# ArthurBrussee/brush

Measured on NVIDIA H100. Metric: fwd+bwd Mpix/s @1M Gaussians 1080p, higher is better.
Workload: dtype f32

## Files before the change

### brush_b200/csrc/api.cu

```cuda
#include <cuda_runtime.h>

#include <algorithm>
#include <cmath>
#include <cstdio>
#include <cstdint>
#include <cstring>
#include <new>

#include "bg_common.cuh"
#include "bg_project.cuh"
#include "bg_dp.cuh"
#include "bg_update.cuh"
#include "bg_refine.cuh"

namespace bg {
cudaError_t launch_project_cull(cudaStream_t, int, bool, const float *, const float *, uint32_t, const BgCamera &,
                                uint32_t, uint32_t, uint32_t, uint32_t, uint32_t *, uint32_t *, uint32_t *, float *,
                                uint32_t *, unsigned long long *, uint32_t *, unsigned long long *, const uint32_t *,
                                uint32_t);
cudaError_t launch_gather_scan(cudaStream_t, int, const uint32_t *, const uint32_t *, uint32_t, const uint32_t *,
                               uint32_t *, uint32_t *, uint32_t, uint32_t *, uint32_t *, unsigned long long *,
                               const uint32_t *, uint32_t);
cudaError_t launch_project_visible_emit(cudaStream_t, int, bool, int, const float *, const float *, const float *,
                                        const uint32_t *, const uint32_t *, const BgCamera &, uint32_t, uint32_t,
                                        float *, uint32_t *, uint32_t *, uint32_t, uint32_t *, const unsigned long long *,
                                        uint32_t *, uint32_t);
cudaError_t launch_tile_offsets(cudaStream_t, int, const uint32_t *, const uint32_t *, uint32_t, uint32_t *);
cudaError_t launch_radix_hist(cudaStream_t, int, const uint32_t *, uint32_t, const uint32_t *, uint32_t, uint32_t,
                              uint32_t *);
cudaError_t launch_onesweep_pass(cudaStream_t, int, const uint32_t *, const uint32_t *, uint32_t *, uint32_t *,
                                 uint32_t, const uint32_t *, uint32_t, uint32_t, const uint32_t *, uint32_t *,
                                 unsigned long long *, unsigned long long *, const uint32_t *, uint32_t);
cudaError_t launch_bump_epoch(cudaStream_t, uint32_t *);
uint64_t sort_max_tiles(uint64_t n);
cudaError_t launch_blend_fwd(cudaStream_t, bool, bool, uint32_t, const float *, const uint32_t *, uint32_t *, const uint32_t *,
                             void *, float *, uint32_t *, uint32_t *, uint32_t, uint32_t, uint32_t, const float *, const float *,
                             float *);
cudaError_t launch_blend_bwd(cudaStream_t, bool, uint32_t, const float *, const uint32_t *, const uint32_t *, const float *,
                             const float *, const uint32_t *, const uint32_t *, float *, unsigned long long *, uint32_t,
                             uint32_t, uint32_t, const float *, const float *, const float *, const float *, float *);
cudaError_t launch_project_bwd(cudaStream_t, bool, int, const float *, const float *, const float *,
                               const uint32_t *, const float *, uint32_t, const BgCamera &, float *, float *, float *,
                               float *, float *);
cudaError_t launch_depth_to_means(cudaStream_t, const uint32_t *, const float *, uint32_t, const BgCamera &, float *);
cudaError_t launch_normal_noise(cudaStream_t, uint64_t, uint64_t, uint64_t, float *);
cudaError_t launch_train_fill_lr(cudaStream_t, float *, float *, uint32_t, float, float, float, float);
cudaError_t launch_loss_reduce(cudaStream_t, const float *, uint32_t, uint32_t, const float *, float *);
cudaError_t launch_min_scale(cudaStream_t, uint32_t, const float *, const float *, uint32_t, float, float *);
cudaError_t launch_fold_min_scale_fwd(cudaStream_t, uint32_t, const float *, const float *, const float *, float *, float *);
// ... 31 lines not shown
    snprintf(g_err, sizeof(g_err), "%s: %s", what, e == cudaSuccess ? "invalid argument" : cudaGetErrorString(e));
}

#define BG_CUDA(call)                          \
    do {                                       \
        cudaError_t e__ = (call);              \
        if (e__ != cudaSuccess) {              \
            set_err(#call, e__);               \
            return BG_ERR_CUDA;                \
        }                                      \
    } while (0)

struct BgContext {
    int device = 0;
    int sm_count = 0;
    uint32_t max_n = 0, max_w = 0, max_h = 0, max_tiles = 0;
    uint32_t max_isect = 0;
    uint32_t *epoch_dev = nullptr;
    uint64_t arena_bytes = 0;
    uint32_t *ctl = nullptr;
    uint32_t *depth_key[2] = {nullptr, nullptr};
    uint32_t *depth_val[2] = {nullptr, nullptr};
    uint32_t *counts = nullptr, *cum = nullptr, *cgid_from_gid = nullptr;
    unsigned long long *hit_masks = nullptr;
    float *projected = nullptr;
    uint32_t *isect_key[2] = {nullptr, nullptr};
    uint32_t *isect_val[2] = {nullptr, nullptr};
    uint32_t *tile_offsets = nullptr;
    uint32_t *live_masks = nullptr, *warp_batches = nullptr;
    unsigned long long *blend_stats = nullptr;
    unsigned long long *lb_scan = nullptr;
    unsigned long long *lb_sort = nullptr;
    uint64_t lb_scan_words = 0, lb_sort_words = 0, lb_sort_tile_words = 0;
    uint32_t *counters_host = nullptr;
    int depth_out = 0, isect_out = 0;
    bool depth_forward = false;
};

enum EpochSlots : uint32_t { EP_PROJECT = 0, EP_DEPTH_SORT = 1 , EP_SCAN = 5, EP_TILE_SORT = 6  };

extern "C" uint32_t bg_abi_version(void) { return BG_ABI_VERSION; }
extern "C" const char *bg_last_error_string(void) { return g_err; }

template <typename T>
static cudaError_t arena_alloc(BgContext *c, T **p, uint64_t count) {
    uint64_t bytes = std::max<uint64_t>(count, 1) * sizeof(T);
    bytes = (bytes + 255) & ~uint64_t(255);
    cudaError_t e = cudaMalloc((void **)p, bytes);
    if (e == cudaSuccess) c->arena_bytes += bytes;
    return e;
}

extern "C" int32_t bg_ctx_destroy(BgContext *c) {
    if (!c) return BG_ERR_NULL;
    cudaSetDevice(c->device);
    void *ptrs[] = {c->ctl, c->depth_key[0], c->depth_key[1], c->depth_val[0], c->depth_val[1], c->counts, c->cum,
                    c->cgid_from_gid, c->hit_masks, c->projected, c->isect_key[0], c->isect_key[1], c->isect_val[0], c->isect_val[1],
                    c->tile_offsets, c->lb_scan, c->lb_sort, c->epoch_dev, c->live_masks, c->warp_batches, c->blend_stats};
    for (void *p : ptrs)
        if (p) cudaFree(p);
    if (c->counters_host) cudaFreeHost(c->counters_host);
    delete c;
    return BG_OK;
}

extern "C" int32_t bg_ctx_create(int32_t device, uint32_t max_splats, uint32_t max_w, uint32_t max_h,
                                 uint64_t max_intersections, BgContext **out_ctx) {
    if (!out_ctx) return BG_ERR_NULL;
    *out_ctx = nullptr;
    if (max_splats == 0 || max_w == 0 || max_h == 0) { set_err("bg_ctx_create: zero capacity", cudaSuccess); return BG_ERR_INVALID; }
    if (max_intersections == 0) max_intersections = std::max<uint64_t>(16ull * max_splats, 1ull << 22);
    if (max_intersections >= (1ull << 31)) { set_err("bg_ctx_create: max_intersections must be < 2^31", cudaSuccess); return BG_ERR_INVALID; }
    BG_CUDA(cudaSetDevice(device));
    BgContext *c = new (std::nothrow) BgContext();
    if (!c) return BG_ERR_CUDA;
    c->device = device;
    c->max_n = max_splats; c->max_w = max_w; c->max_h = max_h;
    c->max_isect = (uint32_t)max_intersections;
    c->max_tiles = ((max_w + TILE_W - 1) / TILE_W) * ((max_h + TILE_W - 1) / TILE_W);
    cudaDeviceProp prop;
    cudaError_t e = cudaGetDeviceProperties(&prop, device);
    if (e != cudaSuccess) { set_err("cudaGetDeviceProperties", e); delete c; return BG_ERR_CUDA; }
    c->sm_count = prop.multiProcessorCount;
    const uint64_t n = max_splats, I = c->max_isect;
    const uint64_t sort_tiles = sort_max_tiles(std::max<uint64_t>(n, I));
    c->lb_sort_tile_words = sort_tiles * 256;
    c->lb_sort_words = c->lb_sort_tile_words + (sort_tiles / 16 + 2) * 256;
    c->lb_scan_words = (n + 255) / 256 + 64;
    bool ok = true;
    ok = ok && arena_alloc(c, &c->ctl, 2 * CTL_WORDS) == cudaSuccess;
    for (int i = 0; i < 2; i++) {
        ok = ok && arena_alloc(c, &c->depth_key[i], n) == cudaSuccess;
        ok = ok && arena_alloc(c, &c->depth_val[i], n) == cudaSuccess;
        ok = ok && arena_alloc(c, &c->isect_key[i], I) == cudaSuccess;
        ok = ok && arena_alloc(c, &c->isect_val[i], I) == cudaSuccess;
    }
    ok = ok && arena_alloc(c, &c->counts, n) == cudaSuccess;
    ok = ok && arena_alloc(c, &c->cum, n) == cudaSuccess;
    ok = ok && arena_alloc(c, &c->cgid_from_gid, n) == cudaSuccess;
    ok = ok && arena_alloc(c, &c->hit_masks, n) == cudaSuccess;
    ok = ok && arena_alloc(c, &c->projected, n * BG_PROJECTED_STRIDE) == cudaSuccess;
    ok = ok && arena_alloc(c, &c->tile_offsets, (uint64_t)c->max_tiles * 2) == cudaSuccess;
    ok = ok && arena_alloc(c, &c->live_masks, (I / 32 + c->max_tiles + 2) * 4) == cudaSuccess;
    ok = ok && arena_alloc(c, &c->warp_batches, (uint64_t)c->max_tiles * 4) == cudaSuccess;
    ok = ok && arena_alloc(c, &c->blend_stats, 4) == cudaSuccess;
    ok = ok && arena_alloc(c, &c->lb_scan, c->lb_scan_words) == cudaSuccess;
    ok = ok && arena_alloc(c, &c->lb_sort, c->lb_sort_words) == cudaSuccess;
    ok = ok && arena_alloc(c, &c->epoch_dev, 1) == cudaSuccess;
    ok = ok && cudaHostAlloc((void **)&c->counters_host, 16 * sizeof(uint32_t), cudaHostAllocDefault) == cudaSuccess;
    if (ok) {
        ok = cudaMemset(c->lb_scan, 0, c->lb_scan_words * 8) == cudaSuccess &&
             cudaMemset(c->lb_sort, 0, c->lb_sort_words * 8) == cudaSuccess &&
             cudaMemset(c->ctl, 0, 2 * CTL_WORDS * 4) == cudaSuccess &&
             cudaMemset(c->epoch_dev, 0, 4) == cudaSuccess;
    }
    if (!ok) {
        set_err("bg_ctx_create: arena allocation", cudaGetLastError());
        bg_ctx_destroy(c);
        return BG_ERR_CUDA;
    }
    memset(c->counters_host, 0, 16 * sizeof(uint32_t));
    *out_ctx = c;
    return BG_OK;
// ... 35 lines not shown
    const int deg = sh_degree_from_k(k);
    if (deg < 0) { set_err("Invalid nr. of sh bases", cudaSuccess); return BG_ERR_INVALID; }
    if (pass < 0 || pass > 2) { set_err("invalid pass", cudaSuccess); return BG_ERR_INVALID; }
    if (cam->camera_model > BG_CAMERA_THIN_PRISM_FISHEYE) return BG_ERR_UNSUPPORTED;
    const bool bwd_info = pass != BG_PASS_FORWARD;
    if (bwd_info && n > 0 && !visible) return BG_ERR_NULL;
    if ((((uintptr_t)transforms) | ((uintptr_t)sh) | ((uintptr_t)raw_opac) | ((uintptr_t)out_img)) & 15u) {
        set_err("bg_render_forward: arrays must be 16-byte aligned (bulk / 128-bit access)", cudaSuccess);
        return BG_ERR_INVALID;
    }
    const uint32_t tiles_x = (w + TILE_W - 1) / TILE_W, tiles_y = (h + TILE_W - 1) / TILE_W;
    const uint32_t num_tiles = tiles_x * tiles_y;
    if (n > c->max_n || num_tiles > c->max_tiles) { set_err("bg_render_forward: exceeds context capacity", cudaSuccess); return BG_ERR_CAPACITY; }
    cudaStream_t s = (cudaStream_t)stream;
    BG_CUDA(cudaSetDevice(c->device));
    c->depth_forward = out_depth != nullptr;

    BG_CUDA(launch_bump_epoch(s, c->epoch_dev));
    BG_CUDA(cudaMemsetAsync(c->ctl, 0, CTL_WORDS * sizeof(uint32_t), s));
    BG_CUDA(cudaMemsetAsync(c->tile_offsets, 0, (size_t)num_tiles * 2 * sizeof(uint32_t), s));
    if (bwd_info && n > 0) BG_CUDA(cudaMemsetAsync(visible, 0, (size_t)n * sizeof(float), s));

    const int pgrid = c->sm_count * 5;
    const int vgrid = c->sm_count * 6;
    uint32_t *counters = c->ctl + CTL_COUNTERS;
    BG_CUDA(launch_project_cull(s, pgrid, mip != 0, transforms, raw_opac, n, *cam, w, h, tiles_x, tiles_y,
                                c->depth_key[0], c->depth_val[0], c->counts, max_radius, c->cgid_from_gid, c->hit_masks, c->ctl,
                                c->lb_scan, c->epoch_dev, EP_PROJECT));
    int dout = 0;
    {
        int32_t r = run_sort(c, s, c->depth_key[0], c->depth_val[0], c->depth_key, c->depth_val, n, counters + 0, 32,
                             c->ctl + CTL_HIST_DEPTH, c->ctl + CTL_TICKETS + TK_DEPTH_HIST, 1, EP_DEPTH_SORT, &dout,
                             true);
        if (r != BG_OK) return r;
    }
    c->depth_out = dout;
    const uint32_t *gid_sorted = c->depth_val[dout];
    BG_CUDA(launch_gather_scan(s, c->sm_count * 2, c->counts, gid_sorted, n, counters + 0, c->cum, counters + 1,
                               c->max_isect, counters + 2, c->ctl + CTL_TICKETS + TK_SCAN, c->lb_scan, c->epoch_dev, EP_SCAN));
    uint32_t bits = 0;
    while (bits < 32 && (num_tiles >> bits) != 0) bits++;
    if (n > 0)
        BG_CUDA(launch_project_visible_emit(s, vgrid, mip != 0, deg, transforms, sh, raw_opac, gid_sorted, c->cum, *cam,
                                            tiles_x, tiles_y, c->projected, c->isect_key[0], c->isect_val[0],
                                            c->max_isect, c->cgid_from_gid, c->hit_masks, c->ctl, bits));
    int iout = 0;
    {
        const uint32_t passes = (bits + 7) / 8;
        const int first_dst = 1;
        int32_t r = run_sort(c, s, c->isect_key[0], c->isect_val[0], c->isect_key, c->isect_val, c->max_isect,
                             counters + 1, bits, c->ctl + CTL_HIST_TILE, c->ctl + CTL_TICKETS + TK_TILE_HIST, first_dst,
                             EP_TILE_SORT, &iout, n > 0 && bits <= 16);
        if (r != BG_OK) return r;
        (void)passes;
    }
    c->isect_out = iout;
    BG_CUDA(launch_tile_offsets(s, c->sm_count * 16, c->isect_key[iout], c->ctl, num_tiles, c->tile_offsets));
    BG_CUDA(launch_blend_fwd(s, bwd_info, pass == BG_PASS_BACKWARD_SMOOTH, num_tiles, c->projected, c->isect_val[iout],
                             c->tile_offsets, gid_sorted, out_img, visible, c->live_masks, c->warp_batches, tiles_x, w, h, bg,
                             reinterpret_cast<const float *>(c->depth_key[dout]), out_depth));
    BG_CUDA(cudaMemcpyAsync(c->counters_host, counters, 4 * sizeof(uint32_t), cudaMemcpyDeviceToHost, s));

    st->projected = c->projected;
    st->compact_gid_from_isect = c->isect_val[iout];
    st->global_from_compact_gid = gid_sorted;
    st->compact_from_global_gid = c->cgid_from_gid;
    st->tile_offsets = c->tile_offsets;
    st->depths = reinterpret_cast<const float *>(c->depth_key[dout]);
// ... 1009 lines not shown
```

### brush_b200/csrc/project.cu

```cuda
#include "bg_project.cuh"

namespace bg {

constexpr int PROJ_THREADS = 256;

struct CullResult {
    bool visible;
    float depth;
    uint32_t tiles;
    float radius;
    unsigned long long mask;
    float mx, my, c00, c01, c11, pt;
    uint32_t min_x, min_y, bbw, ntiles;
};

template <bool MIP, bool DIST>
__device__ __forceinline__ CullResult cull_one(const float *t, float raw_opac, const BgCamera &u, uint32_t img_w,
                                               uint32_t img_h, uint32_t tiles_x, uint32_t tiles_y) {
    CullResult r;
    r.visible = false; r.depth = 0.0f; r.tiles = 0; r.radius = 0.0f; r.mask = 0ull;
    r.mx = r.my = r.c00 = r.c01 = r.c11 = r.pt = 0.0f;
    r.min_x = r.min_y = r.bbw = r.ntiles = 0;
    V3 mean_c = world_to_cam(mk3(t[0], t[1], t[2]), u);
    if (!(is_finite(mean_c) && mean_c.z <= 1.0e10f)) return r;
    if (!in_front<DIST>(mean_c, u)) return r;
    V3 scl = mk3(det_expf(t[7]), det_expf(t[8]), det_expf(t[9]));
    if (!is_finite(scl)) return r;
    Q4 qu; qu.w = t[3]; qu.x = t[4]; qu.y = t[5]; qu.z = t[6];
    float qn = dot(qu, qu);
    if (!(qn >= 1.0e-6f && is_finite(qn))) return r;
    if (!is_finite(raw_opac)) return r;
    Q4 quat = normalize(qu);
    S2 raw_cov = calc_cov2d<DIST>(scl, quat, mean_c, u);
    float comp;
    S2 cov = compensate_cov2d<MIP>(raw_cov, comp);
    float opac = det_sigmoid(raw_opac) * comp;
    if (!is_finite(cov)) return r;
    float mx, my;
    project_mean<DIST>(mean_c, u, mx, my);
    if (!(opac >= 1.0f / 255.0f)) return r;
    float pt = det_logf(opac * 255.0f);
    S2 conic = inverse(cov);
    float ex, ey;
    bbox_extent(conic, pt, ex, ey);
    if (!(ex >= 0.0f && ey >= 0.0f)) return r;
    float wf = (float)img_w, hf = (float)img_h;
    bool on_screen = mx + ex > 0.0f && mx - ex < wf && my + ey > 0.0f && my - ey < hf;
    if (!on_screen) return r;
    TileBox bb = tile_bbox(mx, my, ex, ey, tiles_x, tiles_y);
    r.visible = true;
    r.depth = mean_c.z;
    r.radius = fmaxf(ex / wf, ey / hf);
    r.mx = mx; r.my = my; r.c00 = conic.c00; r.c01 = conic.c01; r.c11 = conic.c11; r.pt = pt;
    r.min_x = bb.min_x; r.min_y = bb.min_y; r.bbw = bb.max_x - bb.min_x;
    r.ntiles = (bb.max_y - bb.min_y) * r.bbw;
    return r;
}

__device__ __forceinline__ void warp_count_tiles(CullResult &r) {
    const uint32_t lane = threadIdx.x & 31u;
    uint32_t incl = r.ntiles;
    for (int o = 1; o < 32; o <<= 1) {
        uint32_t t = __shfl_up_sync(0xffffffffu, incl, o);
        if (lane >= (uint32_t)o) incl += t;
    }
    const uint32_t pre = incl - r.ntiles;
    const uint32_t total = __shfl_sync(0xffffffffu, incl, 31);
    uint32_t hits_count = 0;
    unsigned long long mask = 0ull;
    for (uint32_t base = 0; base < total; base += 32) {
        const uint32_t j = base + lane;
        uint32_t own = 0;
#pragma unroll
        for (int step = 16; step > 0; step >>= 1) {
            uint32_t cand = own + step;
            uint32_t pc = __shfl_sync(0xffffffffu, pre, cand & 31u);
// ... 7 lines not shown
        conic.c11 = __shfl_sync(0xffffffffu, r.c11, own);
        const float pt = __shfl_sync(0xffffffffu, r.pt, own);
        const uint32_t min_x = __shfl_sync(0xffffffffu, r.min_x, own), min_y = __shfl_sync(0xffffffffu, r.min_y, own);
        const uint32_t bbw = __shfl_sync(0xffffffffu, r.bbw, own);
        bool hit = false;
        if (j < total) {
            const uint32_t ry = local / bbw, rx = local - ry * bbw;
            hit = tile_hit(min_x + rx, min_y + ry, mx, my, conic, pt);
        }
        const uint32_t hits = __ballot_sync(0xffffffffu, hit);
        const uint32_t lo = max(pre, base), hi = min(pre + r.ntiles, base + 32u);
        if (hi > lo) {
            const uint32_t sft = lo - base, len = hi - lo;
            const uint32_t seg = (hits >> sft) & (len >= 32u ? 0xffffffffu : ((1u << len) - 1u));
            hits_count += __popc(seg);
            const uint32_t local0 = lo - pre;
            if (local0 < 64u) mask |= (unsigned long long)seg << local0;
        }
    }
    r.tiles = hits_count;
    r.mask = mask;
}

template <bool MIP, bool DIST>
__global__ void __launch_bounds__(PROJ_THREADS)
project_cull_kernel(const float *__restrict__ transforms, const float *__restrict__ raw_opac, uint32_t n,
                    BgCamera u, uint32_t img_w, uint32_t img_h, uint32_t tiles_x, uint32_t tiles_y,
                    uint32_t *__restrict__ depth_keys, uint32_t *__restrict__ gids,
                    uint32_t *__restrict__ counts_by_gid, float *__restrict__ max_radius,
                    uint32_t *__restrict__ cgid_from_gid, unsigned long long *__restrict__ hit_masks,
                    uint32_t *__restrict__ ctl,
                    unsigned long long *__restrict__ lb_state, const uint32_t *__restrict__ epoch_base, uint32_t epoch_off) {
    const uint32_t epoch = ((*epoch_base) * 32u + epoch_off) & 0x3FFFFFFFu;
    __shared__ __align__(128) float s_rows_buf[2][PROJ_THREADS * 10];
    __shared__ __align__(8) unsigned long long s_bar[2];
    __shared__ uint32_t s_scan[33];
    __shared__ uint32_t s_tile, s_tile_next, s_prefix;
    __shared__ uint32_t s_dhist[4 * 256];
    const uint32_t num_tiles = (n + PROJ_THREADS - 1) / PROJ_THREADS;
    if (threadIdx.x == 0) { mbar_init(&s_bar[0], 1); mbar_init(&s_bar[1], 1); }
    for (uint32_t i = threadIdx.x; i < 4 * 256; i += PROJ_THREADS) s_dhist[i] = 0;
    __syncthreads();
    auto issue = [&](uint32_t t, uint32_t b) {
        const uint32_t tb = t * PROJ_THREADS;
        const uint32_t bytes = (min((uint32_t)PROJ_THREADS, n - tb) * 40u) & ~15u;
        mbar_expect_tx(&s_bar[b], bytes);
        tma_bulk_g2s(s_rows_buf[b], transforms + (size_t)tb * 10, bytes, &s_bar[b]);
    };
    if (threadIdx.x == 0) {
        uint32_t t = atomicAdd(&ctl[CTL_TICKETS + TK_PROJECT], 1u);
        s_tile = t;
        if (t < num_tiles) issue(t, 0);
    }
    __syncthreads();
    uint32_t tile = s_tile, buf = 0, phase0 = 0, phase1 = 0;
    while (tile < num_tiles) {
        if (threadIdx.x == 0) {
            uint32_t t = atomicAdd(&ctl[CTL_TICKETS + TK_PROJECT], 1u);
            s_tile_next = t;
            if (t < num_tiles) issue(t, buf ^ 1u);
        }
        const uint32_t base = tile * PROJ_THREADS;
        const uint32_t rows = min((uint32_t)PROJ_THREADS, n - base);
        float *s_rows = s_rows_buf[buf];
        if (buf == 0) { mbar_wait(&s_bar[0], phase0); phase0 ^= 1u; } else { mbar_wait(&s_bar[1], phase1); phase1 ^= 1u; }
        if (threadIdx.x == rows - 1) {
            const uint32_t nf = rows * 10, covered = ((rows * 40u) & ~15u) >> 2;
            for (uint32_t i = covered; i < nf; i++) s_rows[i] = __ldg(transforms + (size_t)base * 10 + i);
        }
        const uint32_t gid = base + threadIdx.x;
        CullResult r;
        r.visible = false; r.depth = 0.0f; r.tiles = 0; r.radius = 0.0f; r.mask = 0ull;
        r.mx = r.my = r.c00 = r.c01 = r.c11 = r.pt = 0.0f;
        r.min_x = r.min_y = r.bbw = r.ntiles = 0;
        if (threadIdx.x < rows) {
            float t[10];
#pragma unroll
            for (int j = 0; j < 10; j++) t[j] = s_rows[threadIdx.x * 10 + j];
            r = cull_one<MIP, DIST>(t, __ldg(raw_opac + gid), u, img_w, img_h, tiles_x, tiles_y);
            max_radius[gid] = r.radius;
            cgid_from_gid[gid] = 0xFFFFFFFFu;
        }
        uint32_t total;
        uint32_t local = block_exclusive_scan(r.visible ? 1u : 0u, s_scan, &total);
        unsigned long long *st = lb_state + tile;
        if (threadIdx.x == 0) lb_store(st, epoch, tile == 0 ? LB_INCLUSIVE : LB_AGGREGATE, total);
        warp_count_tiles(r);
        if (threadIdx.x < 32) {
            uint32_t prefix = (tile == 0) ? 0u : lb_lookback_warp(lb_state, tile, epoch);
            if (threadIdx.x == 0) {
                if (tile != 0) lb_store(st, epoch, LB_INCLUSIVE, prefix + total);
                s_prefix = prefix;
                if (tile == num_tiles - 1) ctl[CTL_COUNTERS + 0] = prefix + total;
            }
        }
        __syncthreads();
        if (r.visible) {
            uint32_t slot = s_prefix + local;
            const uint32_t dk = __float_as_uint(r.depth);
            depth_keys[slot] = dk;
#pragma unroll
            for (int p = 0; p < 4; p++) atomicAdd(&s_dhist[p * 256 + ((dk >> (8 * p)) & 255u)], 1u);
            gids[slot] = gid;
            counts_by_gid[gid] = r.tiles;
            hit_masks[gid] = r.mask;
        }
        tile = s_tile_next;
        buf ^= 1u;
        __syncthreads();
    }
    uint32_t *hist = ctl + CTL_HIST_DEPTH;
    for (uint32_t i = threadIdx.x; i < 4 * 256; i += PROJ_THREADS) {
        const uint32_t c = s_dhist[i];
        if (c) atomicAdd(&hist[i], c);
    }
}

constexpr int SCAN_THREADS = 256, SCAN_ITEMS = 8, SCAN_TILE = SCAN_THREADS * SCAN_ITEMS;

__global__ void __launch_bounds__(SCAN_THREADS)
gather_scan_kernel(const uint32_t *__restrict__ in, const uint32_t *__restrict__ gather_idx ,
                   uint32_t n_host, const uint32_t *__restrict__ n_dev, uint32_t *__restrict__ out,
                   uint32_t *__restrict__ total_out , uint32_t capacity,
                   uint32_t *__restrict__ overflow_flag , uint32_t *__restrict__ ticket,
                   unsigned long long *__restrict__ lb_state, const uint32_t *__restrict__ epoch_base, uint32_t epoch_off) {
    const uint32_t epoch = ((*epoch_base) * 32u + epoch_off) & 0x3FFFFFFFu;
    __shared__ uint32_t s_scan[33];
    __shared__ uint32_t s_tile, s_prefix;
// ... 35 lines not shown
                        tot = capacity;
                    }
                    *total_out = tot;
                }
            }
        }
        __syncthreads();
        const uint32_t off = s_prefix + excl;
#pragma unroll
        for (int i = 0; i < SCAN_ITEMS; i++) {
            uint32_t idx = base + i;
            if (idx < n) out[idx] = off + v[i];
        }
        __syncthreads();
    }
}

constexpr int VIS_THREADS = 128;

__device__ __forceinline__ void prefetch_l2_bulk(const void *p, uint32_t bytes) {
    asm volatile("cp.async.bulk.prefetch.L2.global [%0], %1;" ::"l"(p), "r"(bytes) : "memory");
}

template <bool MIP, int DEG, bool DIST>
__global__ void __launch_bounds__(VIS_THREADS, 6)
project_visible_emit_kernel(const float *__restrict__ transforms, const float *__restrict__ sh,
                            const float *__restrict__ raw_opac, const uint32_t *__restrict__ gid_sorted,
                            const uint32_t *__restrict__ cum, BgCamera u, uint32_t tiles_x, uint32_t tiles_y,
                            float *__restrict__ projected, uint32_t *__restrict__ tile_keys,
                            uint32_t *__restrict__ isect_vals, uint32_t isect_capacity,
                            uint32_t *__restrict__ cgid_from_gid, const unsigned long long *__restrict__ hit_masks,
                            uint32_t *__restrict__ ctl, uint32_t tile_bits) {
    constexpr int KF = (DEG + 1) * (DEG + 1) * 3;
    constexpr bool VEC4 = (KF % 4) == 0;
    constexpr uint32_t EMIT_BUF = 1024;
    __shared__ uint32_t s_emit_keys[(VIS_THREADS / 32) * EMIT_BUF];
    __shared__ uint8_t s_emit_own[(VIS_THREADS / 32) * EMIT_BUF];
    __shared__ uint32_t s_thist[2 * 256];
    const uint32_t hist_passes = (tile_bits <= 16u) ? (tile_bits + 7u) / 8u : 0u;
    const uint32_t hi_mask = (tile_bits > 8u) ? ((1u << min(8u, tile_bits - 8u)) - 1u) : 0u;
    const uint32_t lo_mask = (1u << min(8u, tile_bits)) - 1u;
    for (uint32_t i = threadIdx.x; i < 2 * 256; i += VIS_THREADS) s_thist[i] = 0;
    __syncthreads();
    auto count_key = [&](uint32_t key) {
        if (hist_passes > 0) atomicAdd(&s_thist[key & lo_mask], 1u);
        if (hist_passes > 1) atomicAdd(&s_thist[256 + ((key >> 8) & hi_mask)], 1u);
    };
    const uint32_t nvis = ctl[CTL_COUNTERS + 0];
    const uint32_t num_tickets = (nvis + 31u) / 32u;
    const uint32_t lane = threadIdx.x & 31u, wid = threadIdx.x >> 5;
    const uint32_t lt_mask = (1u << lane) - 1u;
    uint32_t *wkeys = s_emit_keys + wid * EMIT_BUF;
    uint8_t *wown = s_emit_own + wid * EMIT_BUF;
    auto take_ticket = [&]() {
        uint32_t t = 0;
        if (lane == 0) t = atomicAdd(&ctl[CTL_TICKETS + TK_VISIBLE], 1u);
        return __shfl_sync(0xffffffffu, t, 0);
    };
    uint32_t ticket = take_ticket();
    uint32_t gid = 0;
    if (ticket < num_tickets && ticket * 32u + lane < nvis) gid = __ldg(gid_sorted + ticket * 32u + lane);
    while (ticket < num_tickets) {
        const uint32_t cgid = ticket * 32u + lane;
        const bool active = cgid < nvis;
        const uint32_t ticket_next = take_ticket();
        const bool next_active = ticket_next < num_tickets && ticket_next * 32u + lane < nvis;
        uint32_t gid_next = 0;
        if (next_active) gid_next = __ldg(gid_sorted + ticket_next * 32u + lane);

        TileBox bb;
        bb.min_x = bb.min_y = bb.max_x = bb.max_y = 0;
        uint32_t base = 0, budget = 0;
        unsigned long long hitm = 0ull;
        float e_mx = 0.f, e_my = 0.f, e_pt = 0.f;
        S2 e_conic; e_conic.c00 = e_conic.c01 = e_conic.c11 = 0.f;
        if (active) {
            float coef[KF];
            if (VEC4) {
                const float4 *row4 = reinterpret_cast<const float4 *>(sh + (size_t)gid * KF);
#pragma unroll
                for (int i = 0; i < KF / 4; i++) {
                    float4 q = __ldg(row4 + i);
                    coef[4 * i] = q.x; coef[4 * i + 1] = q.y; coef[4 * i + 2] = q.z; coef[4 * i + 3] = q.w;
                }
            } else {
                const float *row = sh + (size_t)gid * KF;
#pragma unroll
                for (int i = 0; i < KF; i++) coef[i] = __ldg(row + i);
            }
            const float2 *t2 = reinterpret_cast<const float2 *>(transforms + (size_t)gid * 10);
            float2 a0 = __ldg(t2), a1 = __ldg(t2 + 1), a2 = __ldg(t2 + 2), a3 = __ldg(t2 + 3), a4 = __ldg(t2 + 4);
            const float ro = __ldg(raw_opac + gid);
            hitm = __ldg(hit_masks + gid);
            base = (cgid == 0) ? 0u : __ldg(cum + cgid - 1);
            budget = __ldg(cum + cgid) - base;
            V3 mean = mk3(a0.x, a0.y, a1.x);
            Q4 qu; qu.w = a1.y; qu.x = a2.x; qu.y = a2.y; qu.z = a3.x;
            V3 scl = mk3(det_expf(a3.y), det_expf(a4.x), det_expf(a4.y));
            Q4 quat = normalize(qu);
            V3 mean_c = world_to_cam(mean, u);
            S2 raw_cov = calc_cov2d<DIST>(scl, quat, mean_c, u);
            float comp;
            S2 cov = compensate_cov2d<MIP>(raw_cov, comp);
            float opac = det_sigmoid(ro) * comp;
            S2 conic = inverse(cov);
            float mx, my;
            project_mean<DIST>(mean_c, u, mx, my);
            V3 vdir = normalize(sub(mean, mk3(u.cam_pos[0], u.cam_pos[1], u.cam_pos[2])));
            V3 raw = sh_to_color<DEG>([&](int i) { return coef[i]; }, vdir);
            float cr = raw.x + 0.5f, cg = raw.y + 0.5f, cb = raw.z + 0.5f;
            cr = clampf(is_finite(cr) ? cr : 0.0f, -100.0f, 100.0f);
            cg = clampf(is_finite(cg) ? cg : 0.0f, -100.0f, 100.0f);
            cb = clampf(is_finite(cb) ? cb : 0.0f, -100.0f, 100.0f);
            float pt = det_logf(opac * 255.0f);
            float4 *dst = reinterpret_cast<float4 *>(projected + (size_t)cgid * BG_PROJECTED_STRIDE);
            const float L2E = 1.4426950408889634f;
            dst[0] = make_float4(mx, my, conic.c00, conic.c01);
            dst[1] = make_float4(conic.c11, opac, cr, cg);
            dst[2] = make_float4(cb, (0.5f * L2E) * conic.c11, (0.5f * L2E) * conic.c00, L2E * conic.c01);
            dst[3] = make_float4(pt, 0.0f, 0.0f, 0.0f);
            cgid_from_gid[gid] = cgid;
            float ex, ey;
            bbox_extent(conic, pt, ex, ey);
            bb = tile_bbox(mx, my, ex, ey, tiles_x, tiles_y);
            e_mx = mx; e_my = my; e_conic = conic; e_pt = pt;
        }
        if (next_active) {
            const char *srow = reinterpret_cast<const char *>(sh + (size_t)gid_next * KF);
            const char *trow = reinterpret_cast<const char *>(transforms + (size_t)gid_next * 10);
            if (VEC4) prefetch_l2_bulk(srow, KF * 4);
            prefetch_l2_bulk(reinterpret_cast<const char *>(reinterpret_cast<uintptr_t>(trow) & ~(uintptr_t)15), 48);
        }
        const uint32_t warp_base = __shfl_sync(0xffffffffu, base, 0);
        uint32_t end_here = active ? base + budget : 0u;
        for (int o = 16; o > 0; o >>= 1) end_here = max(end_here, __shfl_xor_sync(0xffffffffu, end_here, o));
        const uint32_t warp_total = end_here - warp_base;
        const bool staged = warp_total <= EMIT_BUF;
        const uint32_t off = base - warp_base;
        const uint32_t bbw = bb.max_x - bb.min_x, bbh = bb.max_y - bb.min_y;
        const bool big = active && bbw * bbh > 64u;
        auto put = [&](uint32_t slot_off, uint32_t slot_base, uint32_t owner_lane, uint32_t h, uint32_t key) {
            if (staged) { wkeys[slot_off + h] = key; wown[slot_off + h] = (uint8_t)owner_lane; }
            else {
                uint32_t o = slot_base + h;
                if (o < isect_capacity) { tile_keys[o] = key; isect_vals[o] = ticket * 32u + owner_lane; count_key(key); }
            }
        };
        if (active && !big) {
            uint32_t hits = 0;
            unsigned long long m = hitm;
            const unsigned long long row_mask = (bbw >= 64u) ? ~0ull : ((1ull << bbw) - 1ull);
            uint32_t row_key = bb.min_x + bb.min_y * tiles_x;
            for (uint32_t ry = 0; ry < bbh && hits < budget; ry++, m = (bbw >= 64u) ? 0ull : (m >> bbw), row_key += tiles_x) {
                unsigned long long rb = m & row_mask;
                while (rb && hits < budget) {
// ... 77 lines not shown
tile_offsets_kernel(const uint32_t *__restrict__ tile_ids, const uint32_t *__restrict__ ctl, uint32_t num_tiles,
                    uint32_t *__restrict__ tile_offsets) {
    const uint32_t n = ctl[CTL_COUNTERS + 1];
    const uint32_t groups = (n + 3u) / 4u;
    for (uint32_t g = blockIdx.x * blockDim.x + threadIdx.x; g < groups; g += gridDim.x * blockDim.x) {
        const uint32_t i0 = g * 4u;
        uint32_t v[4];
        if (i0 + 4u <= n) {
            const uint4 q = __ldg(reinterpret_cast<const uint4 *>(tile_ids) + g);
            v[0] = q.x; v[1] = q.y; v[2] = q.z; v[3] = q.w;
        } else {
#pragma unroll
            for (int e = 0; e < 4; e++) v[e] = (i0 + e < n) ? __ldg(tile_ids + i0 + e) : 0xFFFFFFFFu;
        }
        uint32_t prev = (i0 == 0) ? 0xFFFFFFFFu : __ldg(tile_ids + i0 - 1);
#pragma unroll
        for (int e = 0; e < 4; e++) {
            if (i0 + e < n) tile_boundary(i0 + e, v[e], prev, n, num_tiles, tile_offsets);
            prev = v[e];
        }
    }
}

cudaError_t launch_project_cull(cudaStream_t s, int grid, bool mip, const float *transforms, const float *raw_opac,
                                uint32_t n, const BgCamera &u, uint32_t w, uint32_t h, uint32_t tx, uint32_t ty,
                                uint32_t *depth_keys, uint32_t *gids, uint32_t *counts, float *max_radius,
                                uint32_t *cgid_from_gid, unsigned long long *hit_masks, uint32_t *ctl,
                                unsigned long long *lb, const uint32_t *epoch_base, uint32_t epoch_off) {
    if (n == 0) return cudaSuccess;
    const bool dist = u.camera_model != BG_CAMERA_PINHOLE;
#define BG_LAUNCH_CULL(M, D)                                                                                       \
    project_cull_kernel<M, D><<<grid, PROJ_THREADS, 0, s>>>(transforms, raw_opac, n, u, w, h, tx, ty, depth_keys, \
                                                            gids, counts, max_radius, cgid_from_gid, hit_masks, ctl, lb, epoch_base, epoch_off)
    if (mip) { if (dist) BG_LAUNCH_CULL(true, true); else BG_LAUNCH_CULL(true, false); }
    else     { if (dist) BG_LAUNCH_CULL(false, true); else BG_LAUNCH_CULL(false, false); }
#undef BG_LAUNCH_CULL
    return cudaGetLastError();
}

cudaError_t launch_gather_scan(cudaStream_t s, int grid, const uint32_t *in, const uint32_t *gather_idx,
                               uint32_t n_host, const uint32_t *n_dev, uint32_t *out, uint32_t *total_out,
                               uint32_t capacity, uint32_t *overflow_flag, uint32_t *ticket,
                               unsigned long long *lb, const uint32_t *epoch_base, uint32_t epoch_off) {
    if (n_host == 0) return cudaSuccess;
    gather_scan_kernel<<<grid, SCAN_THREADS, 0, s>>>(in, gather_idx, n_host, n_dev, out, total_out, capacity,
                                                     overflow_flag, ticket, lb, epoch_base, epoch_off);
    return cudaGetLastError();
}

template <bool MIP>
static cudaError_t launch_visible_deg(cudaStream_t s, int grid, int deg, const float *transforms, const float *sh,
                                      const float *raw_opac, const uint32_t *gid_sorted, const uint32_t *cum,
                                      const BgCamera &u, uint32_t tx, uint32_t ty, float *projected,
                                      uint32_t *tile_keys, uint32_t *isect_vals, uint32_t cap,
                                      uint32_t *cgid_from_gid, const unsigned long long *hit_masks, uint32_t *ctl,
                                      uint32_t tile_bits) {
    const bool dist = u.camera_model != BG_CAMERA_PINHOLE;
#define BG_LAUNCH_VIS(D)                                                                                                   \
    if (dist) project_visible_emit_kernel<MIP, D, true><<<grid, VIS_THREADS, 0, s>>>(transforms, sh, raw_opac, gid_sorted, cum, u, \
                                                                     tx, ty, projected, tile_keys, isect_vals, cap, cgid_from_gid, hit_masks, ctl, tile_bits); \
    else project_visible_emit_kernel<MIP, D, false><<<grid, VIS_THREADS, 0, s>>>(transforms, sh, raw_opac, gid_sorted, cum, u, \
                                                                     tx, ty, projected, tile_keys, isect_vals, cap, cgid_from_gid, hit_masks, ctl, tile_bits)
    switch (deg) {
        case 0: BG_LAUNCH_VIS(0); break;
        case 1: BG_LAUNCH_VIS(1); break;
        case 2: BG_LAUNCH_VIS(2); break;
        case 3: BG_LAUNCH_VIS(3); break;
        case 4: BG_LAUNCH_VIS(4); break;
        default: return cudaErrorInvalidValue;
    }
#undef BG_LAUNCH_VIS
    return cudaGetLastError();
}

cudaError_t launch_project_visible_emit(cudaStream_t s, int grid, bool mip, int deg, const float *transforms,
                                        const float *sh, const float *raw_opac, const uint32_t *gid_sorted,
                                        const uint32_t *cum, const BgCamera &u, uint32_t tx, uint32_t ty,
                                        float *projected, uint32_t *tile_keys, uint32_t *isect_vals, uint32_t cap,
                                        uint32_t *cgid_from_gid, const unsigned long long *hit_masks, uint32_t *ctl,
                                        uint32_t tile_bits) {
    return mip ? launch_visible_deg<true>(s, grid, deg, transforms, sh, raw_opac, gid_sorted, cum, u, tx, ty, projected,
                                          tile_keys, isect_vals, cap, cgid_from_gid, hit_masks, ctl, tile_bits)
               : launch_visible_deg<false>(s, grid, deg, transforms, sh, raw_opac, gid_sorted, cum, u, tx, ty,
                                           projected, tile_keys, isect_vals, cap, cgid_from_gid, hit_masks, ctl, tile_bits);
}

cudaError_t launch_tile_offsets(cudaStream_t s, int grid, const uint32_t *tile_ids, const uint32_t *ctl,
                                uint32_t num_tiles, uint32_t *tile_offsets) {
    tile_offsets_kernel<<<grid, 256, 0, s>>>(tile_ids, ctl, num_tiles, tile_offsets);
    return cudaGetLastError();
}

}
```

Measured before the change: 991.6.

## Compute projected rows and SH color in cull pass, copy in emit

The cull kernel now evaluates SH color for visible splats and writes a full projected row (mean, conic, opacity, color, log-threshold, hit mask) indexed by gid into a new buffer. The emit kernel no longer recomputes covariance, conic and color. It just copies the precomputed row into depth-sorted order and derives the tile bbox from it. This removes the duplicated projection math and the second read of transforms and SH coefficients. In exchange the cull kernel does more work and writes an extra 64-byte row per visible splat. Emit occupancy and grid size are raised from 6 to 8 blocks per SM.

```diff
diff --git a/brush_b200/csrc/api.cu b/brush_b200/csrc/api.cu
--- a/brush_b200/csrc/api.cu
+++ b/brush_b200/csrc/api.cu
@@ -14,17 +14,16 @@
 #include "bg_refine.cuh"
 
 namespace bg {
-cudaError_t launch_project_cull(cudaStream_t, int, bool, const float *, const float *, uint32_t, const BgCamera &,
-                                uint32_t, uint32_t, uint32_t, uint32_t, uint32_t *, uint32_t *, uint32_t *, float *,
-                                uint32_t *, unsigned long long *, uint32_t *, unsigned long long *, const uint32_t *,
-                                uint32_t);
+cudaError_t launch_project_cull(cudaStream_t, int, bool, int, const float *, const float *, const float *, uint32_t,
+                                const BgCamera &, uint32_t, uint32_t, uint32_t, uint32_t, uint32_t *, uint32_t *,
+                                uint32_t *, float *, uint32_t *, float *, uint32_t *, unsigned long long *,
+                                const uint32_t *, uint32_t);
 cudaError_t launch_gather_scan(cudaStream_t, int, const uint32_t *, const uint32_t *, uint32_t, const uint32_t *,
                                uint32_t *, uint32_t *, uint32_t, uint32_t *, uint32_t *, unsigned long long *,
                                const uint32_t *, uint32_t);
-cudaError_t launch_project_visible_emit(cudaStream_t, int, bool, int, const float *, const float *, const float *,
-                                        const uint32_t *, const uint32_t *, const BgCamera &, uint32_t, uint32_t,
-                                        float *, uint32_t *, uint32_t *, uint32_t, uint32_t *, const unsigned long long *,
-                                        uint32_t *, uint32_t);
+cudaError_t launch_project_visible_emit(cudaStream_t, int, const float *, const uint32_t *, const uint32_t *, uint32_t,
+                                        uint32_t, float *, uint32_t *, uint32_t *, uint32_t, uint32_t *, uint32_t *,
+                                        uint32_t);
 cudaError_t launch_tile_offsets(cudaStream_t, int, const uint32_t *, const uint32_t *, uint32_t, uint32_t *);
 cudaError_t launch_radix_hist(cudaStream_t, int, const uint32_t *, uint32_t, const uint32_t *, uint32_t, uint32_t,
                               uint32_t *);
@@ -102,7 +101,7 @@
     uint32_t *depth_key[2] = {nullptr, nullptr};
     uint32_t *depth_val[2] = {nullptr, nullptr};
     uint32_t *counts = nullptr, *cum = nullptr, *cgid_from_gid = nullptr;
-    unsigned long long *hit_masks = nullptr;
+    float *row_by_gid = nullptr;
     float *projected = nullptr;
     uint32_t *isect_key[2] = {nullptr, nullptr};
     uint32_t *isect_val[2] = {nullptr, nullptr};
@@ -135,7 +134,7 @@
     if (!c) return BG_ERR_NULL;
     cudaSetDevice(c->device);
     void *ptrs[] = {c->ctl, c->depth_key[0], c->depth_key[1], c->depth_val[0], c->depth_val[1], c->counts, c->cum,
-                    c->cgid_from_gid, c->hit_masks, c->projected, c->isect_key[0], c->isect_key[1], c->isect_val[0], c->isect_val[1],
+                    c->cgid_from_gid, c->row_by_gid, c->projected, c->isect_key[0], c->isect_key[1], c->isect_val[0], c->isect_val[1],
                     c->tile_offsets, c->lb_scan, c->lb_sort, c->epoch_dev, c->live_masks, c->warp_batches, c->blend_stats};
     for (void *p : ptrs)
         if (p) cudaFree(p);
@@ -178,7 +177,7 @@
     ok = ok && arena_alloc(c, &c->counts, n) == cudaSuccess;
     ok = ok && arena_alloc(c, &c->cum, n) == cudaSuccess;
     ok = ok && arena_alloc(c, &c->cgid_from_gid, n) == cudaSuccess;
-    ok = ok && arena_alloc(c, &c->hit_masks, n) == cudaSuccess;
+    ok = ok && arena_alloc(c, &c->row_by_gid, n * BG_PROJECTED_STRIDE) == cudaSuccess;
     ok = ok && arena_alloc(c, &c->projected, n * BG_PROJECTED_STRIDE) == cudaSuccess;
     ok = ok && arena_alloc(c, &c->tile_offsets, (uint64_t)c->max_tiles * 2) == cudaSuccess;
     ok = ok && arena_alloc(c, &c->live_masks, (I / 32 + c->max_tiles + 2) * 4) == cudaSuccess;
@@ -260,11 +259,11 @@
     if (bwd_info && n > 0) BG_CUDA(cudaMemsetAsync(visible, 0, (size_t)n * sizeof(float), s));
 
     const int pgrid = c->sm_count * 5;
-    const int vgrid = c->sm_count * 6;
+    const int vgrid = c->sm_count * 8;
     uint32_t *counters = c->ctl + CTL_COUNTERS;
-    BG_CUDA(launch_project_cull(s, pgrid, mip != 0, transforms, raw_opac, n, *cam, w, h, tiles_x, tiles_y,
-                                c->depth_key[0], c->depth_val[0], c->counts, max_radius, c->cgid_from_gid, c->hit_masks, c->ctl,
-                                c->lb_scan, c->epoch_dev, EP_PROJECT));
+    BG_CUDA(launch_project_cull(s, pgrid, mip != 0, deg, transforms, sh, raw_opac, n, *cam, w, h, tiles_x, tiles_y,
+                                c->depth_key[0], c->depth_val[0], c->counts, max_radius, c->cgid_from_gid, c->row_by_gid,
+                                c->ctl, c->lb_scan, c->epoch_dev, EP_PROJECT));
     int dout = 0;
     {
         int32_t r = run_sort(c, s, c->depth_key[0], c->depth_val[0], c->depth_key, c->depth_val, n, counters + 0, 32,
@@ -279,9 +278,9 @@
     uint32_t bits = 0;
     while (bits < 32 && (num_tiles >> bits) != 0) bits++;
     if (n > 0)
-        BG_CUDA(launch_project_visible_emit(s, vgrid, mip != 0, deg, transforms, sh, raw_opac, gid_sorted, c->cum, *cam,
-                                            tiles_x, tiles_y, c->projected, c->isect_key[0], c->isect_val[0],
-                                            c->max_isect, c->cgid_from_gid, c->hit_masks, c->ctl, bits));
+        BG_CUDA(launch_project_visible_emit(s, vgrid, c->row_by_gid, gid_sorted, c->cum, tiles_x, tiles_y, c->projected,
+                                            c->isect_key[0], c->isect_val[0], c->max_isect, c->cgid_from_gid, c->ctl,
+                                            bits));
     int iout = 0;
     {
         const uint32_t passes = (bits + 7) / 8;
diff --git a/brush_b200/csrc/project.cu b/brush_b200/csrc/project.cu
--- a/brush_b200/csrc/project.cu
+++ b/brush_b200/csrc/project.cu
@@ -11,6 +11,7 @@
     float radius;
     unsigned long long mask;
     float mx, my, c00, c01, c11, pt;
+    float opac;
     uint32_t min_x, min_y, bbw, ntiles;
 };
 
@@ -19,7 +20,7 @@
                                                uint32_t img_h, uint32_t tiles_x, uint32_t tiles_y) {
     CullResult r;
     r.visible = false; r.depth = 0.0f; r.tiles = 0; r.radius = 0.0f; r.mask = 0ull;
-    r.mx = r.my = r.c00 = r.c01 = r.c11 = r.pt = 0.0f;
+    r.mx = r.my = r.c00 = r.c01 = r.c11 = r.pt = r.opac = 0.0f;
     r.min_x = r.min_y = r.bbw = r.ntiles = 0;
     V3 mean_c = world_to_cam(mk3(t[0], t[1], t[2]), u);
     if (!(is_finite(mean_c) && mean_c.z <= 1.0e10f)) return r;
@@ -51,7 +52,7 @@
     r.visible = true;
     r.depth = mean_c.z;
     r.radius = fmaxf(ex / wf, ey / hf);
-    r.mx = mx; r.my = my; r.c00 = conic.c00; r.c01 = conic.c01; r.c11 = conic.c11; r.pt = pt;
+    r.mx = mx; r.my = my; r.c00 = conic.c00; r.c01 = conic.c01; r.c11 = conic.c11; r.pt = pt; r.opac = opac;
     r.min_x = bb.min_x; r.min_y = bb.min_y; r.bbw = bb.max_x - bb.min_x;
     r.ntiles = (bb.max_y - bb.min_y) * r.bbw;
     return r;
@@ -105,13 +106,38 @@
     r.mask = mask;
 }
 
-template <bool MIP, bool DIST>
-__global__ void __launch_bounds__(PROJ_THREADS)
-project_cull_kernel(const float *__restrict__ transforms, const float *__restrict__ raw_opac, uint32_t n,
+template <int DEG>
+__device__ __forceinline__ V3 splat_color(const float *__restrict__ sh, uint32_t gid, V3 vdir) {
+    constexpr int KF = (DEG + 1) * (DEG + 1) * 3;
+    float coef[KF];
+    if ((KF % 4) == 0) {
+        const float4 *row4 = reinterpret_cast<const float4 *>(sh + (size_t)gid * KF);
+#pragma unroll
+        for (int i = 0; i < KF / 4; i++) {
+            float4 q = __ldg(row4 + i);
+            coef[4 * i] = q.x; coef[4 * i + 1] = q.y; coef[4 * i + 2] = q.z; coef[4 * i + 3] = q.w;
+        }
+    } else {
+        const float *row = sh + (size_t)gid * KF;
+#pragma unroll
+        for (int i = 0; i < KF; i++) coef[i] = __ldg(row + i);
+    }
+    V3 raw = sh_to_color<DEG>([&](int i) { return coef[i]; }, vdir);
+    float cr = raw.x + 0.5f, cg = raw.y + 0.5f, cb = raw.z + 0.5f;
+    cr = clampf(is_finite(cr) ? cr : 0.0f, -100.0f, 100.0f);
+    cg = clampf(is_finite(cg) ? cg : 0.0f, -100.0f, 100.0f);
+    cb = clampf(is_finite(cb) ? cb : 0.0f, -100.0f, 100.0f);
+    return mk3(cr, cg, cb);
+}
+
+template <bool MIP, int DEG, bool DIST>
+__global__ void __launch_bounds__(PROJ_THREADS, DIST ? 0 : 5)
+project_cull_kernel(const float *__restrict__ transforms, const float *__restrict__ sh,
+                    const float *__restrict__ raw_opac, uint32_t n,
                     BgCamera u, uint32_t img_w, uint32_t img_h, uint32_t tiles_x, uint32_t tiles_y,
                     uint32_t *__restrict__ depth_keys, uint32_t *__restrict__ gids,
                     uint32_t *__restrict__ counts_by_gid, float *__restrict__ max_radius,
-                    uint32_t *__restrict__ cgid_from_gid, unsigned long long *__restrict__ hit_masks,
+                    uint32_t *__restrict__ cgid_from_gid, float *__restrict__ row_by_gid,
                     uint32_t *__restrict__ ctl,
                     unsigned long long *__restrict__ lb_state, const uint32_t *__restrict__ epoch_base, uint32_t epoch_off) {
     const uint32_t epoch = ((*epoch_base) * 32u + epoch_off) & 0x3FFFFFFFu;
@@ -154,8 +180,9 @@
         const uint32_t gid = base + threadIdx.x;
         CullResult r;
         r.visible = false; r.depth = 0.0f; r.tiles = 0; r.radius = 0.0f; r.mask = 0ull;
-        r.mx = r.my = r.c00 = r.c01 = r.c11 = r.pt = 0.0f;
+        r.mx = r.my = r.c00 = r.c01 = r.c11 = r.pt = r.opac = 0.0f;
         r.min_x = r.min_y = r.bbw = r.ntiles = 0;
+        float4 *row = reinterpret_cast<float4 *>(row_by_gid + (size_t)gid * BG_PROJECTED_STRIDE);
         if (threadIdx.x < rows) {
             float t[10];
 #pragma unroll
@@ -163,6 +190,14 @@
             r = cull_one<MIP, DIST>(t, __ldg(raw_opac + gid), u, img_w, img_h, tiles_x, tiles_y);
             max_radius[gid] = r.radius;
             cgid_from_gid[gid] = 0xFFFFFFFFu;
+            if (r.visible) {
+                const V3 vdir = normalize(sub(mk3(t[0], t[1], t[2]), mk3(u.cam_pos[0], u.cam_pos[1], u.cam_pos[2])));
+                const V3 col = splat_color<DEG>(sh, gid, vdir);
+                const float L2E = 1.4426950408889634f;
+                row[0] = make_float4(r.mx, r.my, r.c00, r.c01);
+                row[1] = make_float4(r.c11, r.opac, col.x, col.y);
+                row[2] = make_float4(col.z, (0.5f * L2E) * r.c11, (0.5f * L2E) * r.c00, L2E * r.c01);
+            }
         }
         uint32_t total;
         uint32_t local = block_exclusive_scan(r.visible ? 1u : 0u, s_scan, &total);
@@ -186,7 +221,7 @@
             for (int p = 0; p < 4; p++) atomicAdd(&s_dhist[p * 256 + ((dk >> (8 * p)) & 255u)], 1u);
             gids[slot] = gid;
             counts_by_gid[gid] = r.tiles;
-            hit_masks[gid] = r.mask;
+            row[3] = make_float4(r.pt, __uint_as_float((uint32_t)r.mask), __uint_as_float((uint32_t)(r.mask >> 32)), 0.0f);
         }
         tile = s_tile_next;
         buf ^= 1u;
@@ -268,17 +303,12 @@
     asm volatile("cp.async.bulk.prefetch.L2.global [%0], %1;" ::"l"(p), "r"(bytes) : "memory");
 }
 
-template <bool MIP, int DEG, bool DIST>
-__global__ void __launch_bounds__(VIS_THREADS, 6)
-project_visible_emit_kernel(const float *__restrict__ transforms, const float *__restrict__ sh,
-                            const float *__restrict__ raw_opac, const uint32_t *__restrict__ gid_sorted,
-                            const uint32_t *__restrict__ cum, BgCamera u, uint32_t tiles_x, uint32_t tiles_y,
+__global__ void __launch_bounds__(VIS_THREADS, 8)
+project_visible_emit_kernel(const float *__restrict__ row_by_gid, const uint32_t *__restrict__ gid_sorted,
+                            const uint32_t *__restrict__ cum, uint32_t tiles_x, uint32_t tiles_y,
                             float *__restrict__ projected, uint32_t *__restrict__ tile_keys,
                             uint32_t *__restrict__ isect_vals, uint32_t isect_capacity,
-                            uint32_t *__restrict__ cgid_from_gid, const unsigned long long *__restrict__ hit_masks,
-                            uint32_t *__restrict__ ctl, uint32_t tile_bits) {
-    constexpr int KF = (DEG + 1) * (DEG + 1) * 3;
-    constexpr bool VEC4 = (KF % 4) == 0;
+                            uint32_t *__restrict__ cgid_from_gid, uint32_t *__restrict__ ctl, uint32_t tile_bits) {
     constexpr uint32_t EMIT_BUF = 1024;
     __shared__ uint32_t s_emit_keys[(VIS_THREADS / 32) * EMIT_BUF];
     __shared__ uint8_t s_emit_own[(VIS_THREADS / 32) * EMIT_BUF];
@@ -321,62 +351,23 @@
         float e_mx = 0.f, e_my = 0.f, e_pt = 0.f;
         S2 e_conic; e_conic.c00 = e_conic.c01 = e_conic.c11 = 0.f;
         if (active) {
-            float coef[KF];
-            if (VEC4) {
-                const float4 *row4 = reinterpret_cast<const float4 *>(sh + (size_t)gid * KF);
-#pragma unroll
-                for (int i = 0; i < KF / 4; i++) {
-                    float4 q = __ldg(row4 + i);
-                    coef[4 * i] = q.x; coef[4 * i + 1] = q.y; coef[4 * i + 2] = q.z; coef[4 * i + 3] = q.w;
-                }
-            } else {
-                const float *row = sh + (size_t)gid * KF;
-#pragma unroll
-                for (int i = 0; i < KF; i++) coef[i] = __ldg(row + i);
-            }
-            const float2 *t2 = reinterpret_cast<const float2 *>(transforms + (size_t)gid * 10);
-            float2 a0 = __ldg(t2), a1 = __ldg(t2 + 1), a2 = __ldg(t2 + 2), a3 = __ldg(t2 + 3), a4 = __ldg(t2 + 4);
-            const float ro = __ldg(raw_opac + gid);
-            hitm = __ldg(hit_masks + gid);
+            const float4 *src = reinterpret_cast<const float4 *>(row_by_gid + (size_t)gid * BG_PROJECTED_STRIDE);
+            const float4 q0 = __ldg(src), q1 = __ldg(src + 1), q2 = __ldg(src + 2), q3 = __ldg(src + 3);
             base = (cgid == 0) ? 0u : __ldg(cum + cgid - 1);
             budget = __ldg(cum + cgid) - base;
-            V3 mean = mk3(a0.x, a0.y, a1.x);
-            Q4 qu; qu.w = a1.y; qu.x = a2.x; qu.y = a2.y; qu.z = a3.x;
-            V3 scl = mk3(det_expf(a3.y), det_expf(a4.x), det_expf(a4.y));
-            Q4 quat = normalize(qu);
-            V3 mean_c = world_to_cam(mean, u);
-            S2 raw_cov = calc_cov2d<DIST>(scl, quat, mean_c, u);
-            float comp;
-            S2 cov = compensate_cov2d<MIP>(raw_cov, comp);
-            float opac = det_sigmoid(ro) * comp;
-            S2 conic = inverse(cov);
-            float mx, my;
-            project_mean<DIST>(mean_c, u, mx, my);
-            V3 vdir = normalize(sub(mean, mk3(u.cam_pos[0], u.cam_pos[1], u.cam_pos[2])));
-            V3 raw = sh_to_color<DEG>([&](int i) { return coef[i]; }, vdir);
-            float cr = raw.x + 0.5f, cg = raw.y + 0.5f, cb = raw.z + 0.5f;
-            cr = clampf(is_finite(cr) ? cr : 0.0f, -100.0f, 100.0f);
-            cg = clampf(is_finite(cg) ? cg : 0.0f, -100.0f, 100.0f);
-            cb = clampf(is_finite(cb) ? cb : 0.0f, -100.0f, 100.0f);
-            float pt = det_logf(opac * 255.0f);
             float4 *dst = reinterpret_cast<float4 *>(projected + (size_t)cgid * BG_PROJECTED_STRIDE);
-            const float L2E = 1.4426950408889634f;
-            dst[0] = make_float4(mx, my, conic.c00, conic.c01);
-            dst[1] = make_float4(conic.c11, opac, cr, cg);
-            dst[2] = make_float4(cb, (0.5f * L2E) * conic.c11, (0.5f * L2E) * conic.c00, L2E * conic.c01);
-            dst[3] = make_float4(pt, 0.0f, 0.0f, 0.0f);
+            dst[0] = q0;
+            dst[1] = q1;
+            dst[2] = q2;
+            dst[3] = make_float4(q3.x, 0.0f, 0.0f, 0.0f);
             cgid_from_gid[gid] = cgid;
+            hitm = (unsigned long long)__float_as_uint(q3.y) | ((unsigned long long)__float_as_uint(q3.z) << 32);
+            e_mx = q0.x; e_my = q0.y; e_conic.c00 = q0.z; e_conic.c01 = q0.w; e_conic.c11 = q1.x; e_pt = q3.x;
             float ex, ey;
-            bbox_extent(conic, pt, ex, ey);
-            bb = tile_bbox(mx, my, ex, ey, tiles_x, tiles_y);
-            e_mx = mx; e_my = my; e_conic = conic; e_pt = pt;
-        }
-        if (next_active) {
-            const char *srow = reinterpret_cast<const char *>(sh + (size_t)gid_next * KF);
-            const char *trow = reinterpret_cast<const char *>(transforms + (size_t)gid_next * 10);
-            if (VEC4) prefetch_l2_bulk(srow, KF * 4);
-            prefetch_l2_bulk(reinterpret_cast<const char *>(reinterpret_cast<uintptr_t>(trow) & ~(uintptr_t)15), 48);
-        }
+            bbox_extent(e_conic, e_pt, ex, ey);
+            bb = tile_bbox(e_mx, e_my, ex, ey, tiles_x, tiles_y);
+        }
+        if (next_active) prefetch_l2_bulk(row_by_gid + (size_t)gid_next * BG_PROJECTED_STRIDE, BG_PROJECTED_STRIDE * 4);
         const uint32_t warp_base = __shfl_sync(0xffffffffu, base, 0);
         uint32_t end_here = active ? base + budget : 0u;
         for (int o = 16; o > 0; o >>= 1) end_here = max(end_here, __shfl_xor_sync(0xffffffffu, end_here, o));
@@ -500,20 +491,40 @@
     }
 }
 
-cudaError_t launch_project_cull(cudaStream_t s, int grid, bool mip, const float *transforms, const float *raw_opac,
-                                uint32_t n, const BgCamera &u, uint32_t w, uint32_t h, uint32_t tx, uint32_t ty,
-                                uint32_t *depth_keys, uint32_t *gids, uint32_t *counts, float *max_radius,
-                                uint32_t *cgid_from_gid, unsigned long long *hit_masks, uint32_t *ctl,
+template <bool MIP>
+static cudaError_t launch_cull_deg(cudaStream_t s, int grid, int deg, const float *transforms, const float *sh,
+                                   const float *raw_opac, uint32_t n, const BgCamera &u, uint32_t w, uint32_t h,
+                                   uint32_t tx, uint32_t ty, uint32_t *depth_keys, uint32_t *gids, uint32_t *counts,
+                                   float *max_radius, uint32_t *cgid_from_gid, float *row_by_gid, uint32_t *ctl,
+                                   unsigned long long *lb, const uint32_t *epoch_base, uint32_t epoch_off) {
+    const bool dist = u.camera_model != BG_CAMERA_PINHOLE;
+#define BG_LAUNCH_CULL(D)                                                                                                  \
+    if (dist) project_cull_kernel<MIP, D, true><<<grid, PROJ_THREADS, 0, s>>>(transforms, sh, raw_opac, n, u, w, h, tx, ty, \
+                                       depth_keys, gids, counts, max_radius, cgid_from_gid, row_by_gid, ctl, lb, epoch_base, epoch_off); \
+    else project_cull_kernel<MIP, D, false><<<grid, PROJ_THREADS, 0, s>>>(transforms, sh, raw_opac, n, u, w, h, tx, ty,      \
+                                       depth_keys, gids, counts, max_radius, cgid_from_gid, row_by_gid, ctl, lb, epoch_base, epoch_off)
+    switch (deg) {
+        case 0: BG_LAUNCH_CULL(0); break;
+        case 1: BG_LAUNCH_CULL(1); break;
+        case 2: BG_LAUNCH_CULL(2); break;
+        case 3: BG_LAUNCH_CULL(3); break;
+        case 4: BG_LAUNCH_CULL(4); break;
+        default: return cudaErrorInvalidValue;
+    }
+#undef BG_LAUNCH_CULL
+    return cudaGetLastError();
+}
+
+cudaError_t launch_project_cull(cudaStream_t s, int grid, bool mip, int deg, const float *transforms, const float *sh,
+                                const float *raw_opac, uint32_t n, const BgCamera &u, uint32_t w, uint32_t h,
+                                uint32_t tx, uint32_t ty, uint32_t *depth_keys, uint32_t *gids, uint32_t *counts,
+                                float *max_radius, uint32_t *cgid_from_gid, float *row_by_gid, uint32_t *ctl,
                                 unsigned long long *lb, const uint32_t *epoch_base, uint32_t epoch_off) {
     if (n == 0) return cudaSuccess;
-    const bool dist = u.camera_model != BG_CAMERA_PINHOLE;
-#define BG_LAUNCH_CULL(M, D)                                                                                       \
-    project_cull_kernel<M, D><<<grid, PROJ_THREADS, 0, s>>>(transforms, raw_opac, n, u, w, h, tx, ty, depth_keys, \
-                                                            gids, counts, max_radius, cgid_from_gid, hit_masks, ctl, lb, epoch_base, epoch_off)
-    if (mip) { if (dist) BG_LAUNCH_CULL(true, true); else BG_LAUNCH_CULL(true, false); }
-    else     { if (dist) BG_LAUNCH_CULL(false, true); else BG_LAUNCH_CULL(false, false); }
-#undef BG_LAUNCH_CULL
-    return cudaGetLastError();
+    return mip ? launch_cull_deg<true>(s, grid, deg, transforms, sh, raw_opac, n, u, w, h, tx, ty, depth_keys, gids,
+                                       counts, max_radius, cgid_from_gid, row_by_gid, ctl, lb, epoch_base, epoch_off)
+               : launch_cull_deg<false>(s, grid, deg, transforms, sh, raw_opac, n, u, w, h, tx, ty, depth_keys, gids,
+                                        counts, max_radius, cgid_from_gid, row_by_gid, ctl, lb, epoch_base, epoch_off);
 }
 
 cudaError_t launch_gather_scan(cudaStream_t s, int grid, const uint32_t *in, const uint32_t *gather_idx,
@@ -526,41 +537,13 @@
     return cudaGetLastError();
 }
 
-template <bool MIP>
-static cudaError_t launch_visible_deg(cudaStream_t s, int grid, int deg, const float *transforms, const float *sh,
-                                      const float *raw_opac, const uint32_t *gid_sorted, const uint32_t *cum,
-                                      const BgCamera &u, uint32_t tx, uint32_t ty, float *projected,
-                                      uint32_t *tile_keys, uint32_t *isect_vals, uint32_t cap,
-                                      uint32_t *cgid_from_gid, const unsigned long long *hit_masks, uint32_t *ctl,
-                                      uint32_t tile_bits) {
-    const bool dist = u.camera_model != BG_CAMERA_PINHOLE;
-#define BG_LAUNCH_VIS(D)                                                                                                   \
-    if (dist) project_visible_emit_kernel<MIP, D, true><<<grid, VIS_THREADS, 0, s>>>(transforms, sh, raw_opac, gid_sorted, cum, u, \
-                                                                     tx, ty, projected, tile_keys, isect_vals, cap, cgid_from_gid, hit_masks, ctl, tile_bits); \
-    else project_visible_emit_kernel<MIP, D, false><<<grid, VIS_THREADS, 0, s>>>(transforms, sh, raw_opac, gid_sorted, cum, u, \
-                                                                     tx, ty, projected, tile_keys, isect_vals, cap, cgid_from_gid, hit_masks, ctl, tile_bits)
-    switch (deg) {
-        case 0: BG_LAUNCH_VIS(0); break;
-        case 1: BG_LAUNCH_VIS(1); break;
-        case 2: BG_LAUNCH_VIS(2); break;
-        case 3: BG_LAUNCH_VIS(3); break;
-        case 4: BG_LAUNCH_VIS(4); break;
-        default: return cudaErrorInvalidValue;
-    }
-#undef BG_LAUNCH_VIS
+cudaError_t launch_project_visible_emit(cudaStream_t s, int grid, const float *row_by_gid, const uint32_t *gid_sorted,
+                                        const uint32_t *cum, uint32_t tx, uint32_t ty, float *projected,
+                                        uint32_t *tile_keys, uint32_t *isect_vals, uint32_t cap,
+                                        uint32_t *cgid_from_gid, uint32_t *ctl, uint32_t tile_bits) {
+    project_visible_emit_kernel<<<grid, VIS_THREADS, 0, s>>>(row_by_gid, gid_sorted, cum, tx, ty, projected, tile_keys,
+                                                             isect_vals, cap, cgid_from_gid, ctl, tile_bits);
     return cudaGetLastError();
-}
-
-cudaError_t launch_project_visible_emit(cudaStream_t s, int grid, bool mip, int deg, const float *transforms,
-                                        const float *sh, const float *raw_opac, const uint32_t *gid_sorted,
-                                        const uint32_t *cum, const BgCamera &u, uint32_t tx, uint32_t ty,
-                                        float *projected, uint32_t *tile_keys, uint32_t *isect_vals, uint32_t cap,
-                                        uint32_t *cgid_from_gid, const unsigned long long *hit_masks, uint32_t *ctl,
-                                        uint32_t tile_bits) {
-    return mip ? launch_visible_deg<true>(s, grid, deg, transforms, sh, raw_opac, gid_sorted, cum, u, tx, ty, projected,
-                                          tile_keys, isect_vals, cap, cgid_from_gid, hit_masks, ctl, tile_bits)
-               : launch_visible_deg<false>(s, grid, deg, transforms, sh, raw_opac, gid_sorted, cum, u, tx, ty,
-                                           projected, tile_keys, isect_vals, cap, cgid_from_gid, hit_masks, ctl, tile_bits);
 }
 
 cudaError_t launch_tile_offsets(cudaStream_t s, int grid, const uint32_t *tile_ids, const uint32_t *ctl,
```

Measured after the change: 1053 (median of 6 runs). +6.2%, better.
